# fnordware/j2k

Measured on AMD Instinct MI355X. Metric: Mpixels/s encode, 8Kx8K 16-bit RGB, 5 DWT levels; DWT HBM GB/s vs roofline, higher is better.
Workload: dtype f32

## Files before the change

### j2k_amd/csrc/encoder.cpp

```cpp
#include <hip/hip_runtime.h>

#include <dlfcn.h>

#include <algorithm>
#include <atomic>
#include <chrono>
#include <condition_variable>
#include <functional>
#include <future>
#include <cstdio>
#include <cstdlib>
#include <cstring>
#include <memory>
#include <mutex>
#include <thread>
#include <string>
#include <vector>

#include "common.h"
#include "geometry.h"
#include "kernels.h"
#include "tier2.h"
#include "jp2.h"
#include "rate_block.h"
// ... 191 lines not shown
}

struct EncodeOut {
    const void *d_cs = nullptr;
    size_t len = 0;
};

}

hipStream_t j2k_hip::coder_stream(j2k_hip_encoder *e, int i)
{
    if (!e->mqs[i]) HIP_CHECK(hipStreamCreateWithFlags(&e->mqs[i], hipStreamNonBlocking));
    return e->mqs[i];
}

namespace {

#ifdef J2K_T1_COUNTERS
void t1_counters(T1Args &ta)
{
    static unsigned long long *dbg = nullptr;
    if (!dbg) { HIP_CHECK(hipMalloc(reinterpret_cast<void **>(&dbg), kT1Counters * 8)); }
    else {
        unsigned long long h[kT1Counters];
        HIP_CHECK(hipMemcpy(h, dbg, sizeof(h), hipMemcpyDeviceToHost));
        std::fprintf(stderr, "t1 counters (previous launches): planes %llu | significance pass: %llu run, %llu decisions, fixed-point rounds %llu, "
                             "dense halves %llu with %llu stripes written, sparse halves %llu | cleanup pass: %llu run, %llu decisions, dense halves %llu "
                             "with %llu stripes written, sparse halves %llu | sparse sample rounds %llu, scans over the stage limit %llu | "
                             "refinement pass: %llu decisions, stripe pairs written %llu, skipped %llu\n",
                     h[6], h[10], h[14], h[1], h[12], h[0], h[7], h[11], h[15], h[13], h[2], h[8], h[9], h[17], h[16], h[4], h[5]);
        std::fprintf(stderr, "  cleanup stripes that are all run-length-zero over the block's columns (fills): %llu, cleanup halves whose active stripes are all "
                             "of that kind: %llu | refinement stripe pairs by refined samples: 0: %llu; 1-63: %llu; 64-447: %llu; 448-511: %llu; 512: %llu\n",
                     h[48], h[49], h[5], h[50], h[51], h[52], h[53]);
        static const char *const bucket[7] = {"0", "1-2", "3-4", "5-8", "9-16", "17-32", "33-64"};
        for (int t = 0; t < 2; ++t) {
            std::fprintf(stderr, "  %s passes by the busiest column's visited samples (passes / stripes holding one):", t ? "cleanup" : "significance");
            for (int k = 0; k < 7; ++k) std::fprintf(stderr, " %s: %llu / %llu;", bucket[k], h[20 + 14 * t + k], h[27 + 14 * t + k]);
            std::fprintf(stderr, "\n");
        }
    }
    HIP_CHECK(hipMemset(dbg, 0, kT1Counters * 8));
    ta.dbg = dbg;
}
#endif

DwtLevelArgs dwt_level_args(j2k_hip_encoder *e, const Coding &cod, const FrontendArgs &fa, bool fused, size_t f, int l, int tile_row = -1)
{
    const int NL = (int)cod.levels();
    const size_t S = e->stride;
    const size_t plane_bytes = e->plane_elems * sizeof(int32_t) * cod.ncomp;
    uint8_t *const Pf = e->P.p ? e->P.as<uint8_t>() + f * plane_bytes : nullptr;
    uint8_t *const Qf = NL >= 2 ? e->Q.as<uint8_t>() + f * plane_bytes : nullptr;
    uint8_t *const Zf = e->Z.as<uint8_t>() + f * plane_bytes;
    size_t jpos = 0;
    for (int k = 0; k < l; ++k) jpos += e->h_jobs[(size_t)k].size();
    DwtLevelArgs da{};
    da.src = (l & 1) ? (void *)Qf : (void *)Pf; da.src_stride = (long long)S;
    const bool last = l == NL - 1;
    da.ll = last ? (void *)Zf : ((l & 1) ? (void *)Pf : (void *)Qf); da.ll_stride = (long long)S;
    da.z = Zf; da.z_stride = (long long)S;
    da.jobs = e->jobs.as<DwtJob>() + jpos; da.njobs = (int)e->h_jobs[(size_t)l].size();
    da.max_rw = e->lvl_max_rw[(size_t)l]; da.max_rh = e->lvl_max_rh[(size_t)l];
    da.reversible = cod.reversible;
    da.shared_chip = (e->device >= 0 && e->device < kMaxDevices && g_dev[e->device].inflight.load() > 1) ? 1 : 0;
    da.comp_stride = (long long)e->plane_elems;
    if (l == 0 && fused) {
// ... 141 lines not shown
    e->last_levels = NL;
    e->last_fused = fused;
    const bool word_by_modeller = dwt_word && !busy_guard.word;
    if (dwt_word && !word_by_modeller) launch_set_word(dwt_word, dense_seq, s, busy_guard.word, 0u);
    busy_guard.word = nullptr;
    HIP_CHECK(hipEventRecord(e->ev[EV_DWT], s));

    if (F > 1 && (e->seq_frames != F || !e->seq_valid)) {
        e->h_blks_seq.resize(nb);
        for (size_t f = 0; f < F; ++f)
            for (size_t i = 0; i < nb1; ++i) {
                CblkDev d = e->h_blks[i];
                d.coef_off += (unsigned long long)f * cod.ncomp * e->plane_elems;
                d.sym_off += (unsigned long long)f * e->sym_bytes;
                d.out_off += (unsigned long long)f * e->out_bytes;
                e->h_blks_seq[f * nb1 + i] = d;
            }
        e->blks_seq.ensure(nb * sizeof(CblkDev));
        HIP_CHECK(hipMemcpyAsync(e->blks_seq.p, e->h_blks_seq.data(), nb * sizeof(CblkDev), hipMemcpyHostToDevice, s));
        e->seq_frames = F; e->seq_valid = true;
    }
    const CblkDev *dblk = F > 1 ? e->blks_seq.as<CblkDev>() : e->blks.as<CblkDev>();
    uint32_t *meta = e->meta.as<uint32_t>();
    T1Args ta{};
    ta.coef = NL >= 1 ? e->Z.p : e->P.p; ta.stride = (long long)S;
    ta.blks = dblk; ta.nblks = (int)nb; ta.reversible = cod.reversible;
    ta.sym = e->sym.as<uint8_t>(); ta.out = e->out.as<uint8_t>();
    ta.numbps = meta; ta.npasses = meta + nb; ta.len = meta + 2 * nb; ta.nsym = meta + 3 * nb; ta.err = meta + 4 * nb;
    ta.pass_nsym = e->passes.as<uint32_t>();
    ta.pass_nmsedec = reinterpret_cast<int *>(e->passes.as<uint32_t>() + nb * kDevMaxPasses);
    ta.pass_rate = e->passes.as<uint32_t>() + 2 * nb * kDevMaxPasses;
    ta.mq_prio = tn.mq_prio ? 3 : 0;
    ta.sparse = tn.t1_sparse;
#ifdef J2K_MQ_TIMES
    {
        static unsigned long long *dbg = nullptr;
        if (!dbg) { HIP_CHECK(hipMalloc(reinterpret_cast<void **>(&dbg), kT1Counters * 8)); }
        else {
            unsigned long long h[12];
            HIP_CHECK(hipMemcpy(h, dbg, sizeof(h), hipMemcpyDeviceToHost));
            const double ch = (double)std::max(1ull, h[4]), wv = (double)std::max(1ull, h[5]);
            std::fprintf(stderr, "coder waves (previous frame): %.0f workgroups, %.0f chunks each; per chunk of 16 decisions, counter ticks: producer work %.1f + barrier %.1f | "
                                 "consumer work %.1f + barrier %.1f\n", wv, ch / wv, h[0] / ch, h[1] / ch, h[2] / ch, h[3] / ch);
        }
        HIP_CHECK(hipMemset(dbg, 0, kT1Counters * 8));
        ta.dbg = dbg;
    }
#endif
#ifdef J2K_T1_COUNTERS
    t1_counters(ta);
#endif
    ta.yield_word = (dwt_word && tn.mq_yield && tn.overlap) ? dwt_word + 32 : nullptr;
    const bool rate_control = cod.rate_control();
    ta.want_dist = rate_control ? 1 : 0;
    {
        const int big_groups = std::max(2, std::min(7, tn.groups));
        const int groups = nb >= 8192 ? big_groups : 1;
        int first = 0;
        for (int gi = 0; gi < groups; ++gi) {
            const size_t eighth = (nb / 8) / 64 * 64;
            int last = gi == groups - 1 ? (int)nb : (int)((eighth + (nb - eighth) * (size_t)gi / (size_t)(groups - 1)) / 64 * 64);
            T1Args tg = ta;
            tg.first = first; tg.nblks = last;
            if (gi == 0 && word_by_modeller) { tg.done_word = dwt_word; tg.done_value = dense_seq; }
            launch_t1_model(tg, s);
            {
// ... 459 lines not shown
    e->sym.ensure(e->sym_bytes + 1024);
    e->out.ensure(e->out_bytes + 64);
    e->cs.ensure(e->out_bytes + 64);
    e->meta.ensure((4 * nb + 4) * sizeof(uint32_t));
    e->passes.ensure(nb * kDevMaxPasses * 3 * sizeof(uint32_t));
    e->h_meta.ensure((4 * nb + 4) * sizeof(uint32_t));
    uint32_t *meta = e->meta.as<uint32_t>();
    e->gate_state.ensure((NG + (size_t)NS + 8) * sizeof(uint32_t));
    unsigned *const gate_ready = e->gate_state.as<unsigned>(), *const gate_done = gate_ready + NG, *const gate_abort = gate_done + NS;
    HIP_CHECK(hipEventRecord(e->ev[EV_START], s));
    HIP_CHECK(hipMemsetAsync(meta + 4 * nb, 0, sizeof(uint32_t), s));
    HIP_CHECK(hipMemsetAsync(gate_ready, 0, (NG + (size_t)NS + 8) * sizeof(uint32_t), s));
    HIP_CHECK(hipEventRecord(e->gates_zeroed, s));

    j2k_hip_plane dplanes[4];
    for (uint32_t c = 0; c < cod.ncomp; ++c) {
        dplanes[c] = planes[c];
        dplanes[c].base = dbase + (static_cast<const uint8_t *>(planes[c].base) - lo);
    }
    const FrontendArgs fa = make_frontend_args(cod, dplanes, 0, 0, (int)cod.width, (int)cod.height);
    e->last_fa = fa; e->last_fused = true; e->last_levels = NL;
    for (int l = 0; l < NL; ++l) e->level_ms[l] = 0;

    T1Args ta{};
    ta.coef = e->Z.p; ta.stride = (long long)e->stride;
    ta.blks = e->blks_band.as<CblkDev>(); ta.nblks = (int)nb; ta.reversible = cod.reversible;
    ta.sym = e->sym.as<uint8_t>(); ta.out = e->out.as<uint8_t>();
    ta.numbps = meta; ta.npasses = meta + nb; ta.len = meta + 2 * nb; ta.nsym = meta + 3 * nb; ta.err = meta + 4 * nb;
    ta.pass_nsym = e->passes.as<uint32_t>();
    ta.pass_nmsedec = reinterpret_cast<int *>(e->passes.as<uint32_t>() + nb * kDevMaxPasses);
    ta.pass_rate = e->passes.as<uint32_t>() + 2 * nb * kDevMaxPasses;
    ta.mq_prio = tn.mq_prio ? 3 : 0;
    ta.sparse = tn.t1_sparse;
    ta.gate_groups = e->gate_groups.as<T1Args::GateGroup>(); ta.gate_group_of = e->gate_group_of.as<unsigned>();
    ta.gate_ready = gate_ready; ta.gate_done = gate_done; ta.gate_abort = gate_abort;
    ta.gate_budget = 1u << 21;

    double dwt_bytes = 0;
    for (int l = 0; l < NL; ++l)
        for (const DwtJob &j : e->h_jobs[(size_t)l]) dwt_bytes += 8.0 * j.rw * j.rh;

    pd.banded = true;
    HIP_CHECK(hipStreamWaitEvent(s_coder, e->gates_zeroed, 0));
    for (size_t g0 = 0; g0 < NG; g0 += 1024) launch_t1_mq_gated(ta, (int)g0, (int)std::min<size_t>(1024, NG - g0), s_coder);
    double up_ms = 0;
    for (int k = 0; k < NS; ++k) {
        const BandStage &st = S.stages[(size_t)k];
        if (k < B) {
            Range r("j2k_hip upload band");
            const uint8_t *b0 = k ? lo + (size_t)rows[(size_t)k - 1] * (size_t)rowbytes : lo;
            const uint8_t *b1 = k == B - 1 ? hi : std::min(hi, lo + (size_t)rows[(size_t)k] * (size_t)rowbytes);
            const double t0 = now_ms();
            if (b1 > b0) HIP_CHECK(hipMemcpyAsync(dbase + (b0 - lo), b0, (size_t)(b1 - b0), hipMemcpyHostToDevice, e->up_stream));
            up_ms += now_ms() - t0;
            HIP_CHECK(hipEventRecord(e->band_up[k], e->up_stream));
        }
        Range r("j2k_hip band enqueue");
        if (k < B) HIP_CHECK(hipStreamWaitEvent(s, e->band_up[k], 0));
        for (const BandLaunch &bl : st.dwt) {
            DwtLevelArgs da = dwt_level_args(e, cod, fa, true, 0, (int)bl.level, (int)bl.tile_row);
            da.pair0 = bl.pair0; da.pair1 = bl.pair1;
            launch_dwt_level(da, s);
        }
        HIP_CHECK(hipGetLastError());
        if (k < B) {
            HIP_CHECK(hipEventRecord(e->gev[k], s));
// ... 689 lines not shown
            d.stepsize = stepsize ? stepsize[i] : 1.0f;
            d.w = (unsigned short)bw[i]; d.h = (unsigned short)bh[i]; d.orient = (unsigned char)orient[i]; d.Mb = 30;
            sym_off += symcap; out_off += outcap;
            blks[i] = d;
        }
        {
            std::vector<uint32_t> order(nb);
            for (uint32_t i = 0; i < nb; ++i) order[i] = i;
            std::sort(order.begin(), order.end(), [&](uint32_t a, uint32_t b) { return by[a] < by[b]; });
            for (size_t i = 0; i < nb; ++i)
                for (size_t j = i + 1; j < nb && by[order[j]] < by[order[i]] + bh[order[i]]; ++j) {
                    const uint32_t a = order[i], b = order[j];
                    if (bx[a] < bx[b] + bw[b] && bx[b] < bx[a] + bw[a]) throw Error(J2K_HIP_ERR_PARAM, "code-block rectangles overlap");
                }
            for (size_t i = 0; i < nb; ++i)
                if ((uint64_t)bx[i] + bw[i] > stride) throw Error(J2K_HIP_ERR_PARAM, "code-block rectangle wider than the plane's stride");
        }
        e->geo_valid = false;
        e->blks.ensure(std::max<size_t>(1, nb) * sizeof(CblkDev));
        if (nb) HIP_CHECK(hipMemcpyAsync(e->blks.p, blks.data(), nb * sizeof(CblkDev), hipMemcpyHostToDevice, s));
        e->sym.ensure(sym_off + 1024); e->out.ensure(out_off + 64);
        e->meta.ensure((4 * nb + 4) * sizeof(uint32_t));
        e->passes.ensure(std::max<size_t>(1, nb) * kDevMaxPasses * 3 * sizeof(uint32_t));
        uint32_t *meta = e->meta.as<uint32_t>();
        T1Args ta{};
        ta.coef = d_coef; ta.stride = stride; ta.blks = e->blks.as<CblkDev>(); ta.nblks = (int)nb; ta.reversible = reversible;
        ta.sym = e->sym.as<uint8_t>(); ta.out = e->out.as<uint8_t>();
        ta.numbps = meta; ta.npasses = meta + nb; ta.len = meta + 2 * nb; ta.nsym = meta + 3 * nb; ta.err = meta + 4 * nb;
        ta.pass_nsym = e->passes.as<uint32_t>();
        ta.pass_nmsedec = reinterpret_cast<int *>(e->passes.as<uint32_t>() + nb * kDevMaxPasses);
        ta.pass_rate = e->passes.as<uint32_t>() + 2 * nb * kDevMaxPasses;
        ta.want_dist = pass_dist != nullptr;
        ta.sparse = tuning().t1_sparse;
#ifdef J2K_T1_COUNTERS
        t1_counters(ta);
#endif
        HIP_CHECK(hipMemsetAsync(ta.err, 0, sizeof(uint32_t), s));
        launch_t1_model(ta, s);
        launch_t1_mq(ta, s);
        std::vector<uint32_t> hm(4 * nb + 1);
        HIP_CHECK(hipMemcpyAsync(hm.data(), meta, hm.size() * sizeof(uint32_t), hipMemcpyDeviceToHost, s));
        HIP_CHECK(hipStreamSynchronize(s));
        if (hm[4 * nb]) throw Error(J2K_HIP_ERR_OVERFLOW, "Tier-1 kernel reported error " + std::to_string(hm[4 * nb]));
        size_t pos = 0;
        for (size_t i = 0; i < nb; ++i) {
            numbps[i] = hm[i]; npasses[i] = hm[nb + i]; length[i] = hm[2 * nb + i];
            offsets[i] = pos;
            if (pos + length[i] > data_cap) throw Error(J2K_HIP_ERR_OVERFLOW, "data buffer too small");
            if (length[i]) HIP_CHECK(hipMemcpy(static_cast<uint8_t *>(data) + pos, e->out.as<uint8_t>() + blks[i].out_off, length[i], hipMemcpyDeviceToHost));
            pos += length[i];
        }
        if (pass_rate || pass_dist) {
            std::vector<uint32_t> hp(nb * kDevMaxPasses * 3);
            HIP_CHECK(hipMemcpy(hp.data(), e->passes.p, hp.size() * sizeof(uint32_t), hipMemcpyDeviceToHost));
            for (size_t i = 0; i < nb; ++i) {
                const uint32_t np = npasses[i];
                uint32_t *rate = hp.data() + 2 * nb * kDevMaxPasses + i * kDevMaxPasses;
                uint32_t last = length[i];
                for (uint32_t p = np; p > 0;) { --p; if (rate[p] > last) rate[p] = last; else last = rate[p]; }
                const uint8_t *bytes = static_cast<const uint8_t *>(data) + offsets[i];
                for (uint32_t p = 0; p < np; ++p)
                    if (rate[p] > 0 && bytes[rate[p] - 1] == 0xff) --rate[p];
                for (uint32_t p = 0; p < (uint32_t)kDevMaxPasses; ++p) {
                    if (pass_rate) pass_rate[i * kDevMaxPasses + p] = p < np ? rate[p] : 0;
                    if (pass_dist) pass_dist[i * kDevMaxPasses + p] = p < np ? (int32_t)hp[nb * kDevMaxPasses + i * kDevMaxPasses + p] : 0;
                }
// ... 100 lines not shown
```

### j2k_amd/csrc/kernels.h

```cpp
#pragma once

#include <hip/hip_runtime.h>

#include <cstdint>

namespace j2k_hip {

struct Tuning {
    int overlap = 1;
    int no_fuse = 0;
    int level_events = 0;
    int level1_dispatch_events = 1;
    int mq_prio = 1;
    int mq_yield = 2;
    int groups = 2;
    int alloc_threads = 8;
    int rate_dev = 0;
    int rate_dev_scan = 0;
    int mq_wait_us = 1500;
    int dwt_pairs = 2;
    int dwt_ppc = 0;
    int dwt_min_waves = 2048;
    int fused_wpb = 0;
    int fused_ppc = 0;
    int fused_generic = 0;
    int dwt_xcd = 1;
    int t1dec_tail = 1;
    int t1dec_lanes = 1;
    int bands = 0;
    int t1_sparse = 0;
};
Tuning &tuning();
int tune(const char *key, int value);
int get_tune(const char *key, int *value);

struct FrontendArgs {
    const uint8_t *src[4];
    long long colbytes[4], rowbytes[4];
    int sample_bytes[4];
    int src_depth[4];
    int ncomp;
    int width;
    int x0;
    int y0, y1;
    int dst_x0, dst_y0;
    int prec;
    int reversible, mct, promote;
    int interleaved;
    const uint8_t *pixel_base;
    int pixel_bytes;
    int chan_off[4];
    void *dst[4];
    long long dst_stride;
};
void launch_frontend(const FrontendArgs &a, hipStream_t s);

struct DwtJob {
    long long src_off;
    long long ll_off;
    long long z_off;
    int rw, rh;
    int casx, casy;
    int px0, py0;
// ... 17 lines not shown
        int rs;
        int dc;
        int mct;
        int ncomp;
        int promote;
        int src_depth, prec;
    } fe;
};
void launch_dwt_level(const DwtLevelArgs &a, hipStream_t s, hipEvent_t start = nullptr, hipEvent_t stop = nullptr);
int fused_occupancy(bool rev, int ncomp);
void launch_membw(const void *src, void *dst, int w, int h, int rows, int mode, hipStream_t s);

struct CblkDev {
    unsigned long long coef_off;
    unsigned long long sym_off;
    unsigned long long out_off;
    unsigned int sym_cap, out_cap;
    float stepsize;
    unsigned short w, h;
    unsigned char orient, Mb;
    unsigned char pad[2];
};
constexpr int kDevMaxPasses = 96;
constexpr int kT1Counters = 56;
struct T1Args {
    const void *coef; long long stride;
    const CblkDev *blks; int nblks;
    int first;
    int reversible;
    int want_dist;
    int mq_prio;
    int model_prio;
    int sparse;
#if defined(J2K_T1_COUNTERS) || defined(J2K_MQ_TIMES)
    unsigned long long *dbg;
#endif
    unsigned *done_word; unsigned done_value;
    struct GateGroup { unsigned first, count, stage, prio; };
    const GateGroup *gate_groups;
    const unsigned *gate_group_of;
    unsigned *gate_ready, *gate_done;
    const unsigned *gate_abort;
    unsigned gate_budget;
    const unsigned *yield_word;
    uint8_t *sym;
    uint8_t *out;
    unsigned int *numbps, *npasses, *nsym, *len, *err;
    unsigned int *pass_nsym;
    int *pass_nmsedec;
    unsigned int *pass_rate;
};
void launch_t1_model(const T1Args &a, hipStream_t s);
void launch_t1_mq(const T1Args &a, hipStream_t s);
void launch_t1_mq_gated(const T1Args &a, int group_first, int group_count, hipStream_t s);
void launch_wait_count(const unsigned *word, unsigned target, unsigned timeout_us, const unsigned *abort, unsigned *err, hipStream_t s);
void launch_wait_word(const unsigned *word, unsigned target, unsigned timeout_us, hipStream_t s);
void launch_set_word(unsigned *word, unsigned value, hipStream_t s, unsigned *word2 = nullptr, unsigned value2 = 0);
void launch_t1_rate_fixup(const T1Args &a, hipStream_t s);

struct Taken;
struct RateArgs {
    unsigned nblks;
    const double *weight;
    const unsigned char *comp_of;
    const unsigned *numbps, *npasses;
    const int *pass_nmsedec;
// ... 82 lines not shown
```

### j2k_amd/csrc/t1.hip

```cpp
#include "kernels.h"
#include "t1_common.h"

#include <algorithm>
#include <cstdlib>
#include <type_traits>

namespace j2k_hip {
namespace {


constexpr int kFrac = 6;
constexpr int kFlush = 1024;
constexpr int kStageBytes = kFlush + 64 * 10;


__device__ __forceinline__ void set_priority(int p)
{
    if (p >= 3) __builtin_amdgcn_s_setprio(3);
    else if (p == 2) __builtin_amdgcn_s_setprio(2);
    else if (p == 1) __builtin_amdgcn_s_setprio(1);
}

__device__ __forceinline__ unsigned from_left(unsigned v) { return (unsigned)__builtin_amdgcn_update_dpp(0, (int)v, 0x138 , 0xf, 0xf, false); }
__device__ __forceinline__ unsigned from_right(unsigned v) { return (unsigned)__builtin_amdgcn_update_dpp(0, (int)v, 0x130 , 0xf, 0xf, false); }

__device__ __forceinline__ u64 from_left64(u64 v) { return (u64)from_left((unsigned)v) | ((u64)from_left((unsigned)(v >> 32)) << 32); }
__device__ __forceinline__ u64 from_right64(u64 v) { return (u64)from_right((unsigned)v) | ((u64)from_right((unsigned)(v >> 32)) << 32); }

__device__ __forceinline__ unsigned prefix_count_dpp(unsigned cnt, unsigned &total)
{
    int t = (int)cnt;
    t += __builtin_amdgcn_update_dpp(0, t, 0x111, 0xf, 0xf, false);
    t += __builtin_amdgcn_update_dpp(0, t, 0x112, 0xf, 0xf, false);
    t += __builtin_amdgcn_update_dpp(0, t, 0x114, 0xf, 0xf, false);
    t += __builtin_amdgcn_update_dpp(0, t, 0x118, 0xf, 0xf, false);
    t += __builtin_amdgcn_update_dpp(0, t, 0x142, 0xa, 0xf, false);
    t += __builtin_amdgcn_update_dpp(0, t, 0x143, 0xc, 0xf, false);
    total = (unsigned)__builtin_amdgcn_readlane(t, 63);
    return (unsigned)t - cnt;
}

__device__ __forceinline__ unsigned nibble_counts(unsigned v)
{
    const unsigned x = v - ((v >> 1) & 0x55555555u);
    return (x & 0x33333333u) + ((x >> 2) & 0x33333333u);
}

constexpr unsigned kDenseStripe = 103, kSparseHead = 64, kSparseRound = 44;
constexpr unsigned kBurst = 64 * 10;

__device__ __forceinline__ int nmsedec_sig(unsigned m, int bp)
{
    const int i = (int)((m >> bp) & 127u);
    return bp > 0 ? max(0, (3 * i - 144) * 128) : ((i * i + 32) >> 6) * 128;
}
__device__ __forceinline__ int nmsedec_ref(unsigned m, int bp)
{
    const int i = (int)((m >> bp) & 127u);
    if (bp > 0) return i >= 64 ? max(0, (i - 80) * 128) : max(0, (48 - i) * 128);
    return (((i - 64) * (i - 64) + 32) >> 6) * 128;
}

struct PackSel {
    u64 v[256];
    constexpr PackSel() : v()
    {
        for (int e = 0; e < 256; ++e) {
            u64 sel = 0x0c0c0c0c0c0c0c0cull;
            int k = 0;
            for (int r = 0; r < 4; ++r) {
                if ((e >> r) & 1) { sel = (sel & ~(0xffull << (8 * k))) | ((u64)r << (8 * k)); ++k; }
                if ((e >> (4 + r)) & 1) { sel = (sel & ~(0xffull << (8 * k))) | ((u64)(4 + r) << (8 * k)); ++k; }
// ... 91 lines not shown
    int numbps = mx ? (32 - __clz((int)mx)) - kFrac : 0;
    if (numbps < 0) numbps = 0;
    __syncthreads();

    unsigned *pass_nsym = a.pass_nsym + (size_t)b * kDevMaxPasses;
    int *pass_nmsedec = a.pass_nmsedec + (size_t)b * kDevMaxPasses;
    auto report = [&]() {
        if (!a.gate_group_of) return;
        __builtin_amdgcn_fence(__ATOMIC_RELEASE, "agent");
        if (lane == 0) __hip_atomic_fetch_add(a.gate_ready + a.gate_group_of[b], 1u, __ATOMIC_RELEASE, __HIP_MEMORY_SCOPE_AGENT);
    };
    if (numbps == 0 || 3 * numbps - 2 > kDevMaxPasses) {
        if (lane == 0) {
            a.numbps[b] = 0; a.npasses[b] = 0; a.nsym[b] = 0;
            if (numbps) a.err[0] = 1u;
        }
        report();
        return;
    }

    const u64 rows_of_block = h == 64 ? ~(u64)0 : (((u64)1 << h) - 1);
    auto rowmask_now = [&]() -> u64 {
        int wv = w;
        asm volatile("" : "+s"(wv));
        return lane < wv ? rows_of_block : 0;
    };
    const int nstripes = (h + 3) >> 2;
    u64 sigma = 0, mu = 0, pi = 0;
    unsigned fill = 0, flushed = 0;
    unsigned char *symout = a.sym + cb.sym_off;
    const unsigned symcap = cb.sym_cap;
    bool overflow = false;

    auto reserve = [&](unsigned cnt, auto maxc, unsigned &total) -> unsigned {
        (void)maxc;
        const unsigned off = prefix_count_dpp(cnt, total);
        return (fill - flushed) + off;
    };
    auto commit = [&](unsigned total) {
        fill += total;
        if (fill - flushed >= kFlush) {
            __builtin_amdgcn_wave_barrier();
            const uint4 v = *reinterpret_cast<const uint4 *>(&stage[lane * 16]);
            const uint4 r = *reinterpret_cast<const uint4 *>(&stage[kFlush + min(lane, 39) * 16]);
            if (flushed + kFlush <= symcap) *reinterpret_cast<uint4 *>(symout + flushed + lane * 16) = v;
            else overflow = true;
            flushed += kFlush;
            __builtin_amdgcn_wave_barrier();
            unsigned z;
            asm volatile("v_mov_b32 %0, 0" : "=v"(z));
            const uint4 zero = make_uint4(z, z, z, z);
            if (lane < 40) {
                *reinterpret_cast<uint4 *>(&stage[lane * 16]) = r;
                *reinterpret_cast<uint4 *>(&stage[kFlush + lane * 16]) = zero;
            } else *reinterpret_cast<uint4 *>(&stage[lane * 16]) = zero;
            __builtin_amdgcn_wave_barrier();
        }
    };
    auto emit = [&](unsigned base, unsigned cnt, unsigned p0, unsigned p1, unsigned p2) {
        const unsigned t = 0u - base;
        const unsigned al = (base + 3u) & ~3u;
        unsigned *const wp = reinterpret_cast<unsigned *>(stage + al);
        const int e = (int)(base + cnt) - (int)al;
        if (cnt != 0 && al != base) __hip_atomic_fetch_or(wp - 1, __builtin_amdgcn_alignbyte(p0, 0u, t), __ATOMIC_RELAXED, __HIP_MEMORY_SCOPE_WAVEFRONT);
        if (e > 0) __hip_atomic_fetch_or(wp, __builtin_amdgcn_alignbyte(p1, p0, t), __ATOMIC_RELAXED, __HIP_MEMORY_SCOPE_WAVEFRONT);
        if (e > 4) __hip_atomic_fetch_or(wp + 1, __builtin_amdgcn_alignbyte(p2, p1, t), __ATOMIC_RELAXED, __HIP_MEMORY_SCOPE_WAVEFRONT);
        if (e > 8) __hip_atomic_fetch_or(wp + 2, __builtin_amdgcn_alignbyte(0u, p2, t), __ATOMIC_RELAXED, __HIP_MEMORY_SCOPE_WAVEFRONT);
    };

    auto emit4 = [&](unsigned base, unsigned cnt, unsigned p0) {
        const unsigned t = 0u - base;
        const unsigned al = (base + 3u) & ~3u;
        unsigned *const wp = reinterpret_cast<unsigned *>(stage + al);
        const int e = (int)(base + cnt) - (int)al;
        if (cnt != 0 && al != base) __hip_atomic_fetch_or(wp - 1, __builtin_amdgcn_alignbyte(p0, 0u, t), __ATOMIC_RELAXED, __HIP_MEMORY_SCOPE_WAVEFRONT);
        if (e > 0) __hip_atomic_fetch_or(wp, __builtin_amdgcn_alignbyte(0u, p0, t), __ATOMIC_RELAXED, __HIP_MEMORY_SCOPE_WAVEFRONT);
    };

#ifdef J2K_T1_COUNTERS
    unsigned long long dc[kT1Counters] = {};
#define DCNT(i) (++dc[i])
#define DADD(i, n) (dc[i] += (n))
#else
#define DCNT(i) ((void)0)
#define DADD(i, n) ((void)0)
#endif
    auto plane_word = [&](int q) -> u64 {
        if (lane >= w) return 0;
// ... 152 lines not shown
            olo |= (unsigned)__builtin_amdgcn_update_dpp(0, (int)olo, ctrl, rmask, 0xf, false);    \
            ohi |= (unsigned)__builtin_amdgcn_update_dpp(0, (int)ohi, ctrl, rmask, 0xf, false);
            J2K_OR_STEP(0x111, 0xf) J2K_OR_STEP(0x112, 0xf) J2K_OR_STEP(0x114, 0xf) J2K_OR_STEP(0x118, 0xf)
            J2K_OR_STEP(0x142, 0xa) J2K_OR_STEP(0x143, 0xc)
#undef J2K_OR_STEP
            const unsigned act[2] = {(unsigned)__builtin_amdgcn_readlane((int)olo, 63), (unsigned)__builtin_amdgcn_readlane((int)ohi, 63)};
            const bool any_n = __any(N64 != 0);
#ifdef J2K_T1_COUNTERS
            {
                unsigned busiest = (unsigned)__popcll(V64);
                for (int o = 32; o > 0; o >>= 1) busiest = max(busiest, (unsigned)__shfl_xor((int)busiest, o));
                const int bucket = busiest == 0 ? 0 : (busiest <= 2 ? 1 : 32 - __clz((int)busiest - 1));
                const int t0 = pt == 0 ? 20 : 34;
                DCNT(pt == 0 ? 10 : 11);
                DCNT(t0 + bucket);
                DADD(t0 + 7 + bucket, __builtin_popcount(act[0]) + __builtin_popcount(act[1]));
            }
#endif
#pragma unroll 1
            for (int half = 0; half < 2; ++half) {
                unsigned active = act[half];
                if (!active) continue;
                auto hf = [&](u64 m) { return half ? (unsigned)(m >> 32) : (unsigned)m; };
                unsigned rl = 0;
                if (pt != 0) {
                    const u64 in = O | LA | RO;
                    u64 busy = in | (in >> 1);
                    busy |= busy >> 2;
                    busy |= ((A | LA | RA) << 1) | ((O | LO | RO) >> 4);
                    u64 full = V64 & (V64 >> 1);
                    full &= full >> 2;
                    rl = hf(full & ~busy & M0);
                }
                const unsigned bitsh = hf(bits), Nh = hf(A) & ~hf(O), Vh = hf(V64);
                const bool any_rl = __any(rl != 0);
                unsigned fills = 0;
                if (any_rl) {
                    unsigned nof = Nh | (Nh >> 1);
                    nof = (nof | (nof >> 2) | ~rl) & 0x11111111u;
                    int wv = w;
                    asm volatile("" : "+s"(wv));
                    if (lane >= wv) nof = 0;
#define J2K_OR_STEP(ctrl, rmask) nof |= (unsigned)__builtin_amdgcn_update_dpp(0, (int)nof, ctrl, rmask, 0xf, false);
                    J2K_OR_STEP(0x111, 0xf) J2K_OR_STEP(0x112, 0xf) J2K_OR_STEP(0x114, 0xf) J2K_OR_STEP(0x118, 0xf)
                    J2K_OR_STEP(0x142, 0xa) J2K_OR_STEP(0x143, 0xc)
#undef J2K_OR_STEP
                    fills = active & ~(unsigned)__builtin_amdgcn_readlane((int)nof, 63);
                    DADD(48, __builtin_popcount(fills));
                    if (fills == active) DCNT(49);
                }
                bool sparse = false;
                u64 q0 = 0, q1 = 0;
                unsigned sparse_total = 0;
                if (a.sparse >= 0 && !any_rl) {
                    const unsigned dense_cost = kDenseStripe * (unsigned)__builtin_popcount(active);
                    if (a.sparse > 0 || !__any(kSparseHead + kSparseRound * (unsigned)__builtin_popcount(Vh) >= dense_cost)) {
                        const unsigned c = nibble_counts(Vh) + nibble_counts(Nh);
                        const unsigned c0 = c & 0x000f000fu, c1 = (c >> 4) & 0x000f000fu, c2 = (c >> 8) & 0x000f000fu, c3 = (c >> 12) & 0x000f000fu;
                        unsigned t0, t1, t2, t3;
                        const unsigned e0 = prefix_count_dpp(c0, t0), e1 = prefix_count_dpp(c1, t1), e2 = prefix_count_dpp(c2, t2), e3 = prefix_count_dpp(c3, t3);
                        const unsigned a1 = t0 + t1, a2 = a1 + t2, a3 = a2 + t3;
                        const unsigned total = (a3 & 0xffffu) + (a3 >> 16);
                        if (total <= kBurst) {
                            sparse = true;
                            sparse_total = total;
                            DCNT(pt == 0 ? 7 : 8);
                            DADD(pt == 0 ? 14 : 15, total);
                            const unsigned org = (fill - flushed) * 0x10001u + (a3 << 16);
                            q0 = (u64)(e0 + org) | ((u64)(e1 + org + t0) << 32);
                            q1 = (u64)(e2 + org + a1) | ((u64)(e3 + org + a2) << 32);
                        } else DCNT(17);
                    }
                }
                unsigned zb0 = 0, zb1 = 0, zb2 = 0, zb3 = 0, sb0 = 0, sb1 = 0, sb2 = 0, sd = 0;
                if (fills != active) {
                    const unsigned Wm1 = hf(LA << 1), W0 = hf(LA), Wp1 = hf(((LA >> 1) & ~M3) | (LO >> 1));
                    const unsigned Em1 = hf((RO << 1) | ((RA << 1) & M0)), E0 = hf(RO), Ep1 = hf(RO >> 1);
                    const unsigned Up = hf(A << 1), Dn = hf(O >> 1);
                    {
                        unsigned h1 = W0 ^ E0, h2 = W0 & E0, v1 = Up ^ Dn, v2 = Up & Dn;
                        if (orient == 1) { const unsigned t1 = h1, t2 = h2; h1 = v1; h2 = v2; v1 = t1; v2 = t2; }
                        const unsigned p = Wm1 ^ Wp1, q = Wm1 & Wp1, r_ = Em1 ^ Ep1, t = Em1 & Ep1;
                        const unsigned dodd = p ^ r_, dge1 = p | q | r_ | t, dge2 = (p & r_) | q | t;
                        const unsigned deq1 = dodd & ~dge2;
                        const unsigned hz = ~(h1 | h2), vnz = v1 | v2;
                        if (orient == 3) {
                            const unsigned dge3 = (q & (r_ | t)) | (t & p);
                            const unsigned deq2 = dge2 & ~dge3, deq0 = ~dge1;
                            const unsigned hv0 = hz & ~vnz, hv1 = (h1 & ~vnz) | (hz & v1), hvge2 = ~(hv0 | hv1);
                            zb3 = dge3;
                            zb2 = deq2 | (deq1 & ~hv0);
                            zb1 = deq2 | (deq1 & hv0) | (deq0 & hvge2);
                            zb0 = (deq2 & ~hv0) | (deq1 & (hv0 | hvge2)) | (deq0 & hv1);
                        } else {
                            zb3 = h2;
                            zb2 = h1 | (hz & v2);
                            zb1 = (h1 & (vnz | dge1)) | (hz & (v1 | (~vnz & dge2)));
                            zb0 = (h1 & (vnz | ~dge1)) | (hz & (v1 | (~vnz & deq1)));
                        }
                    }
                    if (any_n) {
                        const unsigned cL = hf(from_left64(chi)), cR = hf(from_right64(chi)), cU = hf(chi << 1), cD = hf(chi >> 1);
                        const unsigned Wp = W0 & ~cL, Wn = W0 & cL, Ep = E0 & ~cR, En = E0 & cR;
                        const unsigned Upp = Up & ~cU, Upn = Up & cU, Dnp = Dn & ~cD, Dnn = Dn & cD;
                        const unsigned hp = (Wp & ~En) | (Ep & ~Wn), hn = (Wn & ~Ep) | (En & ~Wp);
                        const unsigned vp = (Upp & ~Dnn) | (Dnp & ~Upn), vn = (Upn & ~Dnp) | (Dnn & ~Upp);
                        const unsigned hnz = hp | hn, vnz = vp | vn;
                        const unsigned same = (hp & vp) | (hn & vn), opp = (hp & vn) | (hn & vp);
                        sb2 = same;
                        sb1 = hnz & ~same;
                        sb0 = (hnz & ~same & ~opp) | (~hnz & vnz);
                        sd = hf(chi) ^ (hn | (~hnz & vn));
                    }
                }
                if (sparse) {
                    unsigned rest = Vh, pos = 0;
                    int cur = -1;
                    while (__any(rest != 0)) {
                        DCNT(9);
                        if (rest) {
                            const int r = __builtin_ctz(rest);
                            rest &= rest - 1;
                            const int st = r >> 2;
                            if (st != cur) pos = (unsigned)((r & 8 ? q1 : q0) >> (((r & 4) << 3) | (r & 16))) & 0xffffu;
                            cur = st;
                            const auto bit = [&](unsigned plane) { return __builtin_amdgcn_ubfe(plane, (unsigned)r, 1u); };
                            stage[pos] = (unsigned char)((((((((bit(zb3) << 1) | bit(zb2)) << 1) | bit(zb1)) << 1) | bit(zb0)) << 1) | bit(bitsh));
                            ++pos;
                            if (bit(Nh)) {
                                stage[pos] = (unsigned char)(0x12u + ((((((bit(sb2) << 1) | bit(sb1)) << 1) | bit(sb0)) << 1) | bit(sd)));
                                ++pos;
                            }
                        }
                    }
                    commit(sparse_total);
                    continue;
                }
                DCNT(pt == 0 ? 12 : 13);
                while (active) {
                    const int sl = __builtin_ctz(active) & ~3;
                    active &= active - 1;
                    if ((fills >> sl) & 1u) {
                        int wv = w;
                        asm volatile("" : "+s"(wv));
                        if (lane < wv) stage[(fill - flushed) + lane] = (unsigned char)(CTX_RL << 1);
                        DADD(15, w);
                        commit((unsigned)w);
                        continue;
                    }
                    DCNT(pt == 0 ? 0 : 2);
                    const unsigned bits4 = (bitsh >> sl) & 0xfu;
                    const unsigned N = (Nh >> sl) & 0xfu;
                    unsigned Vz = (Vh >> sl) & 0xfu;
                    unsigned pc = 0, rlsym = 0;
                    if (pt != 0) {
                        if ((rl >> sl) & 1u) {
                            const int runlen = N ? __ffs((int)N) - 1 : 4;
                            rlsym = (CTX_RL << 1) | (runlen != 4 ? 1u : 0u);
                            pc = 1;
                            Vz = 0;
                            if (runlen != 4) {
                                rlsym |= (((CTX_UNI << 1) | (unsigned)(runlen >> 1)) << 8) | (((CTX_UNI << 1) | (unsigned)(runlen & 1)) << 16);
                                pc = 3;
                                Vz = 0xfu & ~((2u << runlen) - 1u);
                            }
                        }
                    }
                    const u64 sel = DIST ? kPackSel.v[Vz | (N << 4)] : sel_tab[Vz | (N << 4)];
                    const unsigned cnt = pc + (unsigned)__builtin_popcount(Vz) + (unsigned)__builtin_popcount(N);
                    unsigned total;
                    const unsigned base = reserve(cnt, std::integral_constant<int, 10>(), total);
                    unsigned zsym = 0, ssym = 0;
                    if (__any(Vz != 0))
                        zsym = (spread4((zb0 >> sl) & 0xfu) << 1) | (spread4((zb1 >> sl) & 0xfu) << 2) | (spread4((zb2 >> sl) & 0xfu) << 3) |
                               (spread4((zb3 >> sl) & 0xfu) << 4) | spread4(bits4);
                    if (__any(N != 0))
                        ssym = 0x12121212u + (spread4((sb0 >> sl) & 0xfu) << 1) + (spread4((sb1 >> sl) & 0xfu) << 2) +
                               (spread4((sb2 >> sl) & 0xfu) << 3) + spread4((sd >> sl) & 0xfu);
                    {
                        const unsigned c0 = __builtin_amdgcn_perm(ssym, zsym, (unsigned)sel), c1 = __builtin_amdgcn_perm(ssym, zsym, (unsigned)(sel >> 32));
                        const u64 d = (((u64)c1 << 32) | c0) << (8 * pc);
                        emit(base, cnt, (unsigned)d | rlsym, (unsigned)(d >> 32), __builtin_amdgcn_ubfe(c1, 8, 8 * pc));
                        DADD(pt == 0 ? 14 : 15, total);
                        commit(total);
                    }
                }
            }
            sigma = A;
            }
            }
            if (pt == 2) pi = 0;
            if constexpr (DIST) {
#pragma unroll
                for (int o = 32; o > 0; o >>= 1) nm += __shfl_xor(nm, o);
            }
            if (lane == 0) { pass_nsym[pass] = fill; pass_nmsedec[pass] = nm; }
            ++pass;
        }
    }
    __builtin_amdgcn_wave_barrier();
    const unsigned rest = fill - flushed;
    if (lane * 16u < rest) {
        if (flushed + lane * 16u + 16u <= symcap) {
            const uint4 v = *reinterpret_cast<const uint4 *>(&stage[lane * 16]);
            *reinterpret_cast<uint4 *>(symout + flushed + lane * 16) = v;
        } else overflow = true;
    }
#ifdef J2K_T1_COUNTERS
    if (lane == 0 && a.dbg) for (int i = 0; i < kT1Counters; ++i) if (dc[i]) atomicAdd(a.dbg + i, dc[i]);
#endif
    const bool ovf = __any(overflow);
    if (ovf && lane == 0) a.err[0] = 2u;
    if (lane == 0) { a.numbps[b] = (unsigned)numbps; a.npasses[b] = ovf ? 0u : (unsigned)pass; a.nsym[b] = ovf ? 0u : fill; }
    report();
}

__device__ __forceinline__ unsigned ctx_word2(unsigned qe, unsigned idx, unsigned mps) { return (qe << 16) | ((idx | (mps << 6)) << 2) | mps; }
// ... 365 lines not shown
```

### j2k_amd/csrc/tuning.cpp

```cpp
#include <cstdlib>
#include <cstring>
#include <mutex>

#include "kernels.h"

namespace j2k_hip {
namespace {

struct Knob { const char *key; const char *env; int Tuning::*field; };
const Knob kKnobs[] = {
    {"overlap", nullptr, &Tuning::overlap},
    {"no_fuse", "J2K_NO_FUSE", &Tuning::no_fuse},
    {"level_events", "J2K_DWT_LEVEL_EVENTS", &Tuning::level_events},
    {"mq_prio", "J2K_MQ_PRIO", &Tuning::mq_prio},
    {"level1_dispatch_events", "J2K_LEVEL1_DISPATCH_EVENTS", &Tuning::level1_dispatch_events},
    {"groups", "J2K_GROUPS", &Tuning::groups},
    {"mq_wait_us", "J2K_MQ_WAIT_US", &Tuning::mq_wait_us},
    {"dwt_pairs", "J2K_DWT_PAIRS", &Tuning::dwt_pairs},
    {"mq_yield", "J2K_MQ_YIELD", &Tuning::mq_yield},
    {"alloc_threads", "J2K_ALLOC_THREADS", &Tuning::alloc_threads},
    {"rate_dev", "J2K_RATE_DEV", &Tuning::rate_dev},
    {"rate_dev_scan", "J2K_RATE_DEV_SCAN", &Tuning::rate_dev_scan},
    {"dwt_ppc", "J2K_DWT_PPC", &Tuning::dwt_ppc},
    {"dwt_min_waves", "J2K_DWT_MIN_WAVES", &Tuning::dwt_min_waves},
    {"fused_wpb", "J2K_DWT_FUSED_WPB", &Tuning::fused_wpb},
    {"fused_ppc", "J2K_DWT_FUSED_PPC", &Tuning::fused_ppc},
    {"fused_generic", "J2K_DWT_FUSED_GENERIC", &Tuning::fused_generic},
    {"dwt_xcd", "J2K_DWT_XCD", &Tuning::dwt_xcd},
    {"t1dec_lanes", "J2K_T1DEC_LANES", &Tuning::t1dec_lanes},
    {"t1dec_tail", "J2K_T1DEC_TAIL", &Tuning::t1dec_tail},
    {"bands", "J2K_BANDS", &Tuning::bands},
    {"t1_sparse", "J2K_T1_SPARSE", &Tuning::t1_sparse},
};

Tuning g_tuning;
std::once_flag g_once;

void from_env()
{
    for (const Knob &k : kKnobs) {
        if (!k.env) continue;
        const char *v = std::getenv(k.env);
        if (v && *v) g_tuning.*(k.field) = std::atoi(v);
        else if (v && (k.field == &Tuning::no_fuse || k.field == &Tuning::level_events))
            g_tuning.*(k.field) = 1;
    }
    if (std::getenv("J2K_NO_OVERLAP")) g_tuning.overlap = 0;
}

}

Tuning &tuning()
{
    std::call_once(g_once, from_env);
    return g_tuning;
}

int tune(const char *key, int value)
{
    if (!key) return 1;
    Tuning &t = tuning();
    for (const Knob &k : kKnobs)
        if (std::strcmp(k.key, key) == 0) { t.*(k.field) = value; return 0; }
    return 1;
}
// ... 12 lines not shown
```

Measured before the change: 9443.

## Encode two adjacent stripes per iteration in the T1 dense stripe loop

```diff
diff --git a/j2k_amd/csrc/encoder.cpp b/j2k_amd/csrc/encoder.cpp
--- a/j2k_amd/csrc/encoder.cpp
+++ b/j2k_amd/csrc/encoder.cpp
@@ -247,6 +247,8 @@
         std::fprintf(stderr, "  cleanup stripes that are all run-length-zero over the block's columns (fills): %llu, cleanup halves whose active stripes are all "
                              "of that kind: %llu | refinement stripe pairs by refined samples: 0: %llu; 1-63: %llu; 64-447: %llu; 448-511: %llu; 512: %llu\n",
                      h[48], h[49], h[5], h[50], h[51], h[52], h[53]);
+        std::fprintf(stderr, "  dense stripe loop: stripe pairs written %llu (committed in two steps, over the stage limit: %llu), stripes written alone %llu\n",
+                     h[18], h[54], h[19]);
         static const char *const bucket[7] = {"0", "1-2", "3-4", "5-8", "9-16", "17-32", "33-64"};
         for (int t = 0; t < 2; ++t) {
             std::fprintf(stderr, "  %s passes by the busiest column's visited samples (passes / stripes holding one):", t ? "cleanup" : "significance");
@@ -454,6 +456,7 @@
     ta.pass_rate = e->passes.as<uint32_t>() + 2 * nb * kDevMaxPasses;
     ta.mq_prio = tn.mq_prio ? 3 : 0;
     ta.sparse = tn.t1_sparse;
+    ta.pair = tn.t1_pair;
 #ifdef J2K_MQ_TIMES
     {
         static unsigned long long *dbg = nullptr;
@@ -979,6 +982,7 @@
     ta.pass_rate = e->passes.as<uint32_t>() + 2 * nb * kDevMaxPasses;
     ta.mq_prio = tn.mq_prio ? 3 : 0;
     ta.sparse = tn.t1_sparse;
+    ta.pair = tn.t1_pair;
     ta.gate_groups = e->gate_groups.as<T1Args::GateGroup>(); ta.gate_group_of = e->gate_group_of.as<unsigned>();
     ta.gate_ready = gate_ready; ta.gate_done = gate_done; ta.gate_abort = gate_abort;
     ta.gate_budget = 1u << 21;
@@ -1734,6 +1738,7 @@
         ta.pass_rate = e->passes.as<uint32_t>() + 2 * nb * kDevMaxPasses;
         ta.want_dist = pass_dist != nullptr;
         ta.sparse = tuning().t1_sparse;
+        ta.pair = tuning().t1_pair;
 #ifdef J2K_T1_COUNTERS
         t1_counters(ta);
 #endif
diff --git a/j2k_amd/csrc/kernels.h b/j2k_amd/csrc/kernels.h
--- a/j2k_amd/csrc/kernels.h
+++ b/j2k_amd/csrc/kernels.h
@@ -29,6 +29,7 @@
     int t1dec_lanes = 1;
     int bands = 0;
     int t1_sparse = 0;
+    int t1_pair = 0;
 };
 Tuning &tuning();
 int tune(const char *key, int value);
@@ -112,6 +113,7 @@
     int mq_prio;
     int model_prio;
     int sparse;
+    int pair;
 #if defined(J2K_T1_COUNTERS) || defined(J2K_MQ_TIMES)
     unsigned long long *dbg;
 #endif
diff --git a/j2k_amd/csrc/t1.hip b/j2k_amd/csrc/t1.hip
--- a/j2k_amd/csrc/t1.hip
+++ b/j2k_amd/csrc/t1.hip
@@ -38,6 +38,14 @@
     t += __builtin_amdgcn_update_dpp(0, t, 0x143, 0xc, 0xf, false);
     total = (unsigned)__builtin_amdgcn_readlane(t, 63);
     return (unsigned)t - cnt;
+}
+
+template <int N>
+__device__ __forceinline__ unsigned shl_fixed(unsigned v)
+{
+    unsigned r;
+    asm("v_lshlrev_b32 %0, %1, %2" : "=v"(r) : "n"(N), "v"(v));
+    return r;
 }
 
 __device__ __forceinline__ unsigned nibble_counts(unsigned v)
@@ -195,28 +203,25 @@
     const unsigned symcap = cb.sym_cap;
     bool overflow = false;
 
-    auto reserve = [&](unsigned cnt, auto maxc, unsigned &total) -> unsigned {
-        (void)maxc;
-        const unsigned off = prefix_count_dpp(cnt, total);
-        return (fill - flushed) + off;
-    };
     auto commit = [&](unsigned total) {
         fill += total;
         if (fill - flushed >= kFlush) {
+            int ln = lane;
+            asm volatile("" : "+v"(ln));
             __builtin_amdgcn_wave_barrier();
-            const uint4 v = *reinterpret_cast<const uint4 *>(&stage[lane * 16]);
-            const uint4 r = *reinterpret_cast<const uint4 *>(&stage[kFlush + min(lane, 39) * 16]);
-            if (flushed + kFlush <= symcap) *reinterpret_cast<uint4 *>(symout + flushed + lane * 16) = v;
+            const uint4 v = *reinterpret_cast<const uint4 *>(&stage[ln * 16]);
+            const uint4 r = *reinterpret_cast<const uint4 *>(&stage[kFlush + min(ln, 39) * 16]);
+            if (flushed + kFlush <= symcap) *reinterpret_cast<uint4 *>(symout + flushed + ln * 16) = v;
             else overflow = true;
             flushed += kFlush;
             __builtin_amdgcn_wave_barrier();
             unsigned z;
             asm volatile("v_mov_b32 %0, 0" : "=v"(z));
             const uint4 zero = make_uint4(z, z, z, z);
-            if (lane < 40) {
-                *reinterpret_cast<uint4 *>(&stage[lane * 16]) = r;
-                *reinterpret_cast<uint4 *>(&stage[kFlush + lane * 16]) = zero;
-            } else *reinterpret_cast<uint4 *>(&stage[lane * 16]) = zero;
+            if (ln < 40) {
+                *reinterpret_cast<uint4 *>(&stage[ln * 16]) = r;
+                *reinterpret_cast<uint4 *>(&stage[kFlush + ln * 16]) = zero;
+            } else *reinterpret_cast<uint4 *>(&stage[ln * 16]) = zero;
             __builtin_amdgcn_wave_barrier();
         }
     };
@@ -435,7 +440,12 @@
                     full &= full >> 2;
                     rl = hf(full & ~busy & M0);
                 }
-                const unsigned bitsh = hf(bits), Nh = hf(A) & ~hf(O), Vh = hf(V64);
+                auto hf_now = [&](u64 m) -> unsigned {
+                    int hv = half;
+                    asm volatile("" : "+s"(hv));
+                    return hv ? (unsigned)(m >> 32) : (unsigned)m;
+                };
+                const unsigned Nh = hf(A) & ~hf(O);
                 const bool any_rl = __any(rl != 0);
                 unsigned fills = 0;
                 if (any_rl) {
@@ -457,8 +467,8 @@
                 unsigned sparse_total = 0;
                 if (a.sparse >= 0 && !any_rl) {
                     const unsigned dense_cost = kDenseStripe * (unsigned)__builtin_popcount(active);
-                    if (a.sparse > 0 || !__any(kSparseHead + kSparseRound * (unsigned)__builtin_popcount(Vh) >= dense_cost)) {
-                        const unsigned c = nibble_counts(Vh) + nibble_counts(Nh);
+                    if (a.sparse > 0 || !__any(kSparseHead + kSparseRound * (unsigned)__builtin_popcount(hf_now(V64)) >= dense_cost)) {
+                        const unsigned c = nibble_counts(hf_now(V64)) + nibble_counts(Nh);
                         const unsigned c0 = c & 0x000f000fu, c1 = (c >> 4) & 0x000f000fu, c2 = (c >> 8) & 0x000f000fu, c3 = (c >> 12) & 0x000f000fu;
                         unsigned t0, t1, t2, t3;
                         const unsigned e0 = prefix_count_dpp(c0, t0), e1 = prefix_count_dpp(c1, t1), e2 = prefix_count_dpp(c2, t2), e3 = prefix_count_dpp(c3, t3);
@@ -517,7 +527,8 @@
                     }
                 }
                 if (sparse) {
-                    unsigned rest = Vh, pos = 0;
+                    const unsigned bitsh = hf(bits);
+                    unsigned rest = hf_now(V64), pos = 0;
                     int cur = -1;
                     while (__any(rest != 0)) {
                         DCNT(9);
@@ -540,52 +551,99 @@
                     continue;
                 }
                 DCNT(pt == 0 ? 12 : 13);
-                while (active) {
-                    const int sl = __builtin_ctz(active) & ~3;
-                    active &= active - 1;
-                    if ((fills >> sl) & 1u) {
-                        int wv = w;
-                        asm volatile("" : "+s"(wv));
-                        if (lane < wv) stage[(fill - flushed) + lane] = (unsigned char)(CTX_RL << 1);
-                        DADD(15, w);
-                        commit((unsigned)w);
-                        continue;
-                    }
-                    DCNT(pt == 0 ? 0 : 2);
-                    const unsigned bits4 = (bitsh >> sl) & 0xfu;
+                auto write_fill = [&]() {
+                    int wv = w;
+                    asm volatile("" : "+s"(wv));
+                    if (lane < wv) stage[(fill - flushed) + lane] = (unsigned char)(CTX_RL << 1);
+                    DADD(15, w);
+                    commit((unsigned)w);
+                };
+                auto column = [&](int sl, unsigned &rlpc) -> unsigned {
                     const unsigned N = (Nh >> sl) & 0xfu;
-                    unsigned Vz = (Vh >> sl) & 0xfu;
-                    unsigned pc = 0, rlsym = 0;
+                    unsigned Vz = (hf_now(V64) >> sl) & 0xfu, pc = 0;
+                    rlpc = 0;
                     if (pt != 0) {
                         if ((rl >> sl) & 1u) {
                             const int runlen = N ? __ffs((int)N) - 1 : 4;
-                            rlsym = (CTX_RL << 1) | (runlen != 4 ? 1u : 0u);
+                            rlpc = (8u << 24) | (CTX_RL << 1) | (runlen != 4 ? 1u : 0u);
                             pc = 1;
                             Vz = 0;
                             if (runlen != 4) {
-                                rlsym |= (((CTX_UNI << 1) | (unsigned)(runlen >> 1)) << 8) | (((CTX_UNI << 1) | (unsigned)(runlen & 1)) << 16);
+                                rlpc |= (16u << 24) | (((CTX_UNI << 1) | (unsigned)(runlen >> 1)) << 8) | (((CTX_UNI << 1) | (unsigned)(runlen & 1)) << 16);
                                 pc = 3;
                                 Vz = 0xfu & ~((2u << runlen) - 1u);
                             }
                         }
                     }
-                    const u64 sel = DIST ? kPackSel.v[Vz | (N << 4)] : sel_tab[Vz | (N << 4)];
-                    const unsigned cnt = pc + (unsigned)__builtin_popcount(Vz) + (unsigned)__builtin_popcount(N);
-                    unsigned total;
-                    const unsigned base = reserve(cnt, std::integral_constant<int, 10>(), total);
-                    unsigned zsym = 0, ssym = 0;
-                    if (__any(Vz != 0))
-                        zsym = (spread4((zb0 >> sl) & 0xfu) << 1) | (spread4((zb1 >> sl) & 0xfu) << 2) | (spread4((zb2 >> sl) & 0xfu) << 3) |
-                               (spread4((zb3 >> sl) & 0xfu) << 4) | spread4(bits4);
-                    if (__any(N != 0))
-                        ssym = 0x12121212u + (spread4((sb0 >> sl) & 0xfu) << 1) + (spread4((sb1 >> sl) & 0xfu) << 2) +
-                               (spread4((sb2 >> sl) & 0xfu) << 3) + spread4((sd >> sl) & 0xfu);
+                    const unsigned idx = Vz | (N << 4);
+                    return idx | ((pc + (unsigned)__builtin_popcount(idx)) << 16);
+                };
+                auto pick = [&](unsigned idx, unsigned zsym, unsigned ssym, unsigned &c0, unsigned &c1) {
+                    const u64 sel = DIST ? kPackSel.v[idx] : sel_tab[idx];
+                    c0 = __builtin_amdgcn_perm(ssym, zsym, (unsigned)sel);
+                    c1 = __builtin_amdgcn_perm(ssym, zsym, (unsigned)(sel >> 32));
+                };
+                auto shift_emit = [&](unsigned base, unsigned cnt, unsigned c0, unsigned c1, unsigned rlpc) {
+                    const unsigned sh = rlpc >> 24;
+                    const u64 d = (((u64)c1 << 32) | c0) << sh;
+                    emit(base, cnt, (unsigned)d | (rlpc & 0xffffffu), (unsigned)(d >> 32), __builtin_amdgcn_ubfe(c1, 8, sh));
+                };
+                auto rows_of_planes = [&](unsigned p0, unsigned p1, unsigned p2, unsigned p3, unsigned k) -> unsigned {
+                    const unsigned sel01 = 0x0c0c0400u + k * 0x0101u, sel23 = 0x04000c0cu + k * 0x01010000u;
+                    unsigned g = __builtin_amdgcn_perm(p1, p0, sel01) | __builtin_amdgcn_perm(p3, p2, sel23);
+                    unsigned t = ((g >> 7) ^ g) & 0x00aa00aau;
+                    g ^= t ^ shl_fixed<7>(t);
+                    t = ((g >> 14) ^ g) & 0x0000ccccu;
+                    g ^= t ^ shl_fixed<14>(t);
+                    return g;
+                };
+                while (active) {
+                    const int s4 = __builtin_ctz(active);
+                    if ((fills >> s4) & 1u) {
+                        active &= active - 1;
+                        write_fill();
+                        continue;
+                    }
+                    const int sl = s4 & ~7;
+                    const bool onA = (s4 & 4) == 0;
+                    const bool onB = !onA || (a.pair >= 0 && (((active & ~fills) >> (sl + 4)) & 1u) != 0);
+                    active &= ~(((onA ? 0x1u : 0u) | (onB ? 0x10u : 0u)) << sl);
                     {
-                        const unsigned c0 = __builtin_amdgcn_perm(ssym, zsym, (unsigned)sel), c1 = __builtin_amdgcn_perm(ssym, zsym, (unsigned)(sel >> 32));
-                        const u64 d = (((u64)c1 << 32) | c0) << (8 * pc);
-                        emit(base, cnt, (unsigned)d | rlsym, (unsigned)(d >> 32), __builtin_amdgcn_ubfe(c1, 8, 8 * pc));
-                        DADD(pt == 0 ? 14 : 15, total);
-                        commit(total);
+                        DADD(pt == 0 ? 0 : 2, onA && onB ? 2 : 1);
+                        DCNT(onA && onB ? 18 : 19);
+                        unsigned meta = 0, rlpcA = 0, rlpcB = 0;
+                        if (onA) meta = column(sl, rlpcA);
+                        if (onB) meta |= column(sl + 4, rlpcB) << 8;
+                        unsigned totals;
+                        const unsigned cnts = __builtin_amdgcn_perm(0u, meta, 0x0c030c02u);
+                        const unsigned offs = prefix_count_dpp(cnts, totals) + (cnts << 11);
+                        unsigned total0 = totals & 0xffffu;
+                        const unsigned total1 = totals >> 16;
+                        unsigned tz, u, ts;
+                        asm("" : "=v"(tz), "=v"(u), "=v"(ts));
+                        const unsigned k = (unsigned)sl >> 3;
+                        if (__any((meta & 0x0f0fu) != 0)) {
+                            tz = rows_of_planes(zb0, zb1, zb2, zb3, k);
+                            const unsigned y = __builtin_amdgcn_ubfe(hf_now(bits), (unsigned)sl, 8u);
+                            u = (y | shl_fixed<7>(y) | shl_fixed<14>(y) | shl_fixed<21>(y)) & 0x11111111u;
+                        }
+                        if (__any((meta & 0xf0f0u) != 0))
+                            ts = rows_of_planes(sd, sb0, sb1, sb2, k);
+                        unsigned c0A, c1A, c0B, c1B;
+                        asm("" : "=v"(c0A), "=v"(c1A), "=v"(c0B), "=v"(c1B));
+                        if (onA) pick(meta & 0xffu, ((tz & 0x0f0f0f0fu) << 1) | (u & 0x01010101u), (ts & 0x0f0f0f0fu) + 0x12121212u, c0A, c1A);
+                        if (onB)
+                            pick(__builtin_amdgcn_ubfe(meta, 8u, 8u), ((tz >> 3) & 0x1e1e1e1eu) | ((u >> 4) & 0x01010101u),
+                                 ((ts >> 4) & 0x0f0f0f0fu) + 0x12121212u, c0B, c1B);
+                        if (onA) shift_emit((fill - flushed) + (offs & 0x7ffu), __builtin_amdgcn_ubfe(offs, 11u, 5u), c0A, c1A, rlpcA);
+                        DADD(pt == 0 ? 14 : 15, total0 + total1);
+                        if (total0 + total1 > kBurst) {
+                            DCNT(54);
+                            commit(total0);
+                            total0 = 0;
+                        }
+                        if (onB) shift_emit((fill - flushed) + total0 + __builtin_amdgcn_ubfe(offs, 16u, 11u), offs >> 27, c0B, c1B, rlpcB);
+                        commit(total0 + total1);
                     }
                 }
             }
diff --git a/j2k_amd/csrc/tuning.cpp b/j2k_amd/csrc/tuning.cpp
--- a/j2k_amd/csrc/tuning.cpp
+++ b/j2k_amd/csrc/tuning.cpp
@@ -31,6 +31,7 @@
     {"t1dec_tail", "J2K_T1DEC_TAIL", &Tuning::t1dec_tail},
     {"bands", "J2K_BANDS", &Tuning::bands},
     {"t1_sparse", "J2K_T1_SPARSE", &Tuning::t1_sparse},
+    {"t1_pair", "J2K_T1_PAIR", &Tuning::t1_pair},
 };
 
 Tuning g_tuning;
```

Result: no change. 9462 (median of 4 runs) (+0.2%).
